# AlwinEsch/pvr.rtl.radiofm

Hardware: AMD Instinct MI355X
Metric: IQ MS/s demodulated (whole node) + achieved HBM GB/s on FIR stage (higher is better)
Workload: dtype f32

## Files before the change

### pvr.rtl.radiofm_amd/csrc/fmd_audio_tail.inc

```
  __builtin_amdgcn_s_setprio(3);
  const unsigned lane = threadIdx.x;
  const unsigned c0 = (blockIdx.x * blockDim.y + threadIdx.y) * 64 + lane;
  if (c0 - lane >= CP)
    return;
  const bool active = c0 < C;
  const unsigned c = active ? c0 : C - 1;
#ifdef FMD_TAIL_ROWS
  const int sel_row = FMD_TAIL_ROWS[c];
  const bool deliver = active && sel_row >= 0;
  const unsigned row = deliver ? (unsigned)sel_row : 0u;
  constexpr bool all_take = false;
#else
  const bool deliver = active;
  const unsigned row = c;
  constexpr bool all_take = true;
#endif
  float de_re = st.F(F_DE_RE)[c], de_im = st.F(F_DE_IM)[c];
  float w1a = st.F(F_N_W1A)[c], w2a = st.F(F_N_W2A)[c], w1b = st.F(F_N_W1B)[c], w2b = st.F(F_N_W2B)[c];
  const int stereo = st.I(I_STEREO_Q0 + (int)stereo_q)[c];
  const float one_minus_alpha = 1.0f - k.de_alpha;
  float vsum = 0.0f, vsumsq = 0.0f;

  auto frame = [&](float2 v) -> float2 {
    de_re = one_minus_alpha * de_re + k.de_alpha * v.x;
    const float s0 = de_re * 2.0f;
    de_im = one_minus_alpha * de_im + k.de_alpha * v.y;
    const float m0 = de_im * 2.0f;
    const float w0a = s0 - k.n_a1 * w1a - k.n_a2 * w2a;
    const float w0b = m0 - k.n_a1 * w1b - k.n_a2 * w2b;
    const float s = k.n_b0 * w0a + k.n_b1 * w1a + k.n_b2 * w2a;
    const float m = k.n_b0 * w0b + k.n_b1 * w1b + k.n_b2 * w2b;
    w2a = w1a;
    w1a = w0a;
    w2b = w1b;
    w1b = w0b;
    const float mm = m * 0.5f;
    const float2 o = stereo ? make_float2((m + s) * 0.5f, (m - s) * 0.5f) : make_float2(mm, mm);
    vsum += o.x;
    vsumsq += o.x * o.x;
    vsum += o.y;
    vsumsq += o.y * o.y;
    return o;
  };
  typename OUT::frame_t* __restrict__ o = reinterpret_cast<typename OUT::frame_t*>(audio + (size_t)row * audio_stride);
  typename OUT::State os;

  unsigned i0 = 0;
  float2 vnext[AT_STEPS];
#pragma unroll
  for (unsigned u = 0; u < AT_STEPS; u++)
    vnext[u] = lp[(size_t)min(u, A - 1) * CP + c];
  for (; i0 + AT_STEPS <= A; i0 += AT_STEPS)
  {
    float2 vin[AT_STEPS];
#pragma unroll
    for (unsigned u = 0; u < AT_STEPS; u++)
      vin[u] = vnext[u];
#pragma unroll
    for (unsigned u = 0; u < AT_STEPS; u++)
      vnext[u] = lp[(size_t)min(i0 + AT_STEPS + u, A - 1) * CP + c];
#pragma unroll
    for (unsigned u = 0; u < AT_STEPS; u++)
    {
      const float2 f = frame(vin[u]);
#ifdef FMD_TAIL_FEED
      if (active)
        FMD_TAIL_FEED[(size_t)(i0 + u) * CP + c] = (f.x + f.y) * 0.5f;
#endif
      if (all_take || deliver)
        OUT::take(os, u, f);
      if (deliver)
        OUT::store(o, os, i0, u, f);
    }
  }
  if (i0 < A)
  {
    const unsigned cnt = A - i0;
#pragma unroll
    for (unsigned u = 0; u < AT_STEPS; u++)
      if (u < cnt)
      {
        const float2 f = frame(vnext[u]);
#ifdef FMD_TAIL_FEED
        if (active)
          FMD_TAIL_FEED[(size_t)(i0 + u) * CP + c] = (f.x + f.y) * 0.5f;
#endif
        if (all_take || deliver)
          OUT::take(os, u, f);
        if (deliver)
          OUT::store(o, os, i0, u, f);
      }
    OUT::flush(o, os, i0, cnt, deliver);
  }
  if (active)
  {
    st.F(F_DE_RE)[c] = de_re;
    st.F(F_DE_IM)[c] = de_im;
    st.F(F_N_W1A)[c] = w1a;
    st.F(F_N_W2A)[c] = w2a;
    st.F(F_N_W1B)[c] = w1b;
    st.F(F_N_W2B)[c] = w2b;
    const float n = (float)(2u * A);
    const float rms = sqrtf(vsumsq / n);
    const float mean = vsum / n;
    const float level = (float)(0.95 * (double)st.F(F_AUDIO_LEVEL)[c] + 0.05 * (double)rms);
    st.F(F_AUDIO_MEAN)[c] = mean;
    st.F(F_AUDIO_RMS)[c] = rms;
    st.F(F_AUDIO_LEVEL)[c] = level;
    unsigned* __restrict__ h = st.ds + c;
    const size_t CPs = st.CP;
    h[HS_IF_LEVEL * CPs] = __float_as_uint(st.F(F_IF_LEVEL)[c]);
    h[HS_BB_MEAN * CPs] = __float_as_uint(st.F(F_BB_MEAN)[c]);
    h[HS_BB_LEVEL * CPs] = __float_as_uint(st.F(F_BB_LEVEL)[c]);
    h[HS_P_LEVEL * CPs] = __float_as_uint(st.F(F_P_LEVEL)[c]);
    h[HS_STEREO * CPs] = (unsigned)stereo;
    h[HS_AUDIO_MEAN * CPs] = __float_as_uint(mean);
    h[HS_AUDIO_RMS * CPs] = __float_as_uint(rms);
    h[HS_AUDIO_LEVEL * CPs] = __float_as_uint(level);
    if (all_take || deliver)
      OUT::done(os, c FMD_TAIL_DONE_ARGS);
  }
```

### pvr.rtl.radiofm_amd/csrc/fmd_k_rds.hip.h

```cpp
#pragma once

#include "fmd_k_common.hip.h"

namespace fmd
{

struct HbCoef
{
  float c[52];
  float e[28];
};

#ifndef FMD_HB_R
#define FMD_HB_R 4
#endif
constexpr int HB_R = FMD_HB_R;

__global__ __launch_bounds__(256) void k_halfband(const float2* __restrict__ in,
                                                  float2* __restrict__ out, unsigned n_out, int L,
                                                  HbCoef hc, unsigned C, unsigned CP, unsigned Hout)
{
  const unsigned c = blockIdx.x * 64 + threadIdx.x;
  const unsigned wy = (unsigned)__builtin_amdgcn_readfirstlane((int)threadIdx.y);
  const unsigned k0 = (blockIdx.y * blockDim.y + wy) * HB_R;
// ... 636 lines not shown
    for (int r = 0; r < RR; r++)
      rf_acc(acc[r], taps[s + r], x);
  }
  if (store)
  {
#pragma unroll
    for (int r = 0; r < RR; r++)
      out[(size_t)(Hout + i + r) * CP + c] = acc[r];
  }
}

template <int RR, typename E>
__device__ __forceinline__ void ring_dispatch(unsigned take, const E* __restrict__ in,
                                              E* __restrict__ out, unsigned i, int T,
                                              const float* __restrict__ taps, unsigned g0, unsigned c,
                                              unsigned CP, unsigned Hout, bool store)
{
  if (take == (unsigned)RR)
    ring_group<RR, E>(in, out, i, T, taps, g0, c, CP, Hout, store);
  else if constexpr (RR > 1)
    ring_dispatch<RR - 1, E>(take, in, out, i, T, taps, g0, c, CP, Hout, store);
}

template <typename E>
__global__ __launch_bounds__(256) void k_ring_fir4(const E* __restrict__ in, E* __restrict__ out,
                                                   unsigned n, int T, const float* __restrict__ taps,
                                                   unsigned g0, unsigned C, unsigned CP, unsigned Hout,
                                                   unsigned prio)
{
  wave_prio(prio);
  const unsigned c = blockIdx.x * 64 + threadIdx.x;
  const unsigned y = (unsigned)__builtin_amdgcn_readfirstlane((int)threadIdx.y);
  unsigned i = (blockIdx.y * blockDim.y + y) * RG;
  if (i >= n)
    return;
  const bool store = c < C;
  unsigned left = min((unsigned)RG, n - i);
  while (left)
  {
    const unsigned room = (unsigned)T - (g0 + i) % (unsigned)T;
    const unsigned take = min(left, room);
    ring_dispatch<RG, E>(take, in, out, i, T, taps, g0, c, CP, Hout, store);
    i += take;
    left -= take;
  }
}

template <typename E>
__global__ __launch_bounds__(256) void k_ring_fir4_org(const E* __restrict__ in, E* __restrict__ out,
                                                       unsigned n, int T, const float* __restrict__ taps,
                                                       unsigned g0, unsigned C, unsigned CP, unsigned Hout,
                                                       unsigned prio, const unsigned* __restrict__ origin)
{
  wave_prio(prio);
  const unsigned c = blockIdx.x * 64 + threadIdx.x;
  const unsigned y = (unsigned)__builtin_amdgcn_readfirstlane((int)threadIdx.y);
  unsigned i = (blockIdx.y * blockDim.y + y) * RG;
  if (i >= n)
    return;
  const bool store = c < C;
  unsigned left = min((unsigned)RG, n - i);
  unsigned lane_g0 = g0;
  const int wg0 = ring_wave_g0(origin, c, C, g0, T, &lane_g0);
  if (wg0 < 0)
  {
    for (; left; i++, left--)
    {
      const unsigned a0 = (lane_g0 + i) % (unsigned)T;
      const E* __restrict__ now = in + (size_t)((unsigned)T - 1 + i) * CP + c;
      const E acc = ring_one_mixed<E>(now, CP, a0, T, taps);
      if (store)
        out[(size_t)(Hout + i) * CP + c] = acc;
    }
    return;
  }
  g0 = (unsigned)wg0;
  while (left)
  {
    const unsigned room = (unsigned)T - (g0 + i) % (unsigned)T;
    const unsigned take = min(left, room);
    ring_dispatch<RG, E>(take, in, out, i, T, taps, g0, c, CP, Hout, store);
    i += take;
    left -= take;
  }
}

template <bool OBS = false>
__device__ __forceinline__ uint32_t rds_check_block(uint32_t& in_bits, uint32_t offset, bool fec,
                                                    uint32_t* pre = nullptr, unsigned* flips = nullptr)
{
  const uint32_t parckh[16] = {0x2DC, 0x16E, 0x0B7, 0x287, 0x39F, 0x313, 0x355, 0x376,
                               0x1BB, 0x201, 0x3DC, 0x1EE, 0x0F7, 0x2A7, 0x38F, 0x31B};
  uint32_t tb = 0x3FFFFFF & in_bits;
  uint32_t syn = tb >> 16;
#pragma unroll
  for (int i = 0; i < 16; i++)
  {
    if (tb & 0x8000)
      syn ^= parckh[i];
    tb <<= 1;
  }
  syn ^= offset;
  if constexpr (OBS)
    *pre = syn;
  if (syn && fec)
  {
    uint32_t mask = 1u << 25;
    for (int i = 0; i < 16; i++)
    {
      if (syn & 0x200)
      {
        if ((syn & 0x1F) == 0)
        {
          in_bits ^= mask;
          syn <<= 1;
          if constexpr (OBS)
            (*flips)++;
        }
        else
        {
          syn <<= 1;
          syn ^= 0x5B9;
        }
      }
      else
        syn <<= 1;
      mask >>= 1;
    }
    syn &= 0x3FF;
  }
  return syn;
}

#ifndef FMD_RP_WAVES
#define FMD_RP_WAVES 4
#endif
constexpr int RP_WAVES = FMD_RP_WAVES;
__global__ __launch_bounds__(64 * RP_WAVES) void k_rds_pll(const float2* __restrict__ lpf, unsigned R, unsigned C,
                                                unsigned CP, RdsConsts k, ChannelState st,
                                                float* __restrict__ rpll, unsigned Hout,
                                                const double* __restrict__ sctab_g, FmdSincosTab sct)
{
  __shared__ double sctab[2 * FMD_SINCOS_TAB_SIZE];
  __builtin_amdgcn_s_setprio(3);
  for (unsigned i = threadIdx.y * 64 + threadIdx.x; i < 2 * FMD_SINCOS_TAB_SIZE; i += 64 * RP_WAVES)
    sctab[i] = sctab_g[i];
  __syncthreads();
  const unsigned c = (blockIdx.x * RP_WAVES + threadIdx.y) * 64 + threadIdx.x;
  if (c >= C)
    return;
  float phase = st.F(F_R_PHASE)[c], freq = st.F(F_R_FREQ)[c];
  float* __restrict__ o = rpll + (size_t)Hout * CP + c;
  constexpr unsigned PT = 16;
  float2 nxt[PT];
#pragma unroll
  for (unsigned u = 0; u < PT; u++)
    nxt[u] = lpf[(size_t)min(u, R - 1) * CP + c];
  for (unsigned i0 = 0; i0 < R; i0 += PT)
  {
    float2 cur[PT];
#pragma unroll
    for (unsigned u = 0; u < PT; u++)
      cur[u] = nxt[u];
#pragma unroll
    for (unsigned u = 0; u < PT; u++)
      nxt[u] = lpf[(size_t)min(i0 + PT + u, R - 1) * CP + c];
    const unsigned cnt = min(PT, R - i0);
#pragma unroll
    for (unsigned u = 0; u < PT; u++)
    {
      if (u < cnt)
      {
        const float2 in = cur[u];
        float sn, cs;
        fmd_sincos_tab(phase, sctab, sct, &sn, &cs);
        const float tr = cs * in.x - sn * in.y;
        const float ti = cs * in.y + sn * in.x;
        const float err = -fmd_rds_arctan2(ti, tr);
        freq += (k.pll_beta * err);
        freq = (freq > k.nco_hl) ? k.nco_hl : ((freq < k.nco_ll) ? k.nco_ll : freq);
        phase += (freq + k.pll_alpha * err);
        *o = ti;
        o += CP;
      }
    }
  }
  st.F(F_R_PHASE)[c] = fmodf(phase, (float)FMD_K_2PI);
  st.F(F_R_FREQ)[c] = freq;
}

constexpr int RB_TILE = 32;

enum RdsQuality
{
  RQ_BITS,
  RQ_CANDIDATES,
  RQ_BLOCKS,
  RQ_CORRECTED,
  RQ_FAILED,
  RQ_ACQUIRED,
  RQ_LOST,
  RQ_GROUPS,
  RQ_N
};
struct RdsObs
{
  unsigned* quality = nullptr;
  uint4* blocks = nullptr;
  unsigned* block_count = nullptr;
  unsigned block_cap = 0;
};

__global__ __launch_bounds__(256) void k_rds_bits(const float* __restrict__ mf, unsigned R, unsigned C,
                                                 unsigned CP, RdsConsts k, ChannelState st,
                                                 uint32_t call_index, RdsGroupRec* __restrict__ queue,
                                                 unsigned* __restrict__ queue_count, unsigned queue_cap,
                                                 float* __restrict__ tap_sync, int write_taps)
{
  constexpr int OBS = 0;
  const RdsObs ob{};
#include "fmd_rds_bits.inc"
}

template <bool RECORD>
__global__ __launch_bounds__(256) void k_rds_bits_obs(const float* __restrict__ mf, unsigned R, unsigned C,
                                                     unsigned CP, RdsConsts k, ChannelState st,
                                                     uint32_t call_index, RdsGroupRec* __restrict__ queue,
                                                     unsigned* __restrict__ queue_count, unsigned queue_cap,
                                                     float* __restrict__ tap_sync, int write_taps, RdsObs ob)
{
  constexpr int OBS = RECORD ? 2 : 1;
#include "fmd_rds_bits.inc"
}

}
```

### pvr.rtl.radiofm_amd/csrc/fmd_k_tail.hip.h

```cpp
#pragma once

#include "fmd_k_common.hip.h"

namespace fmd
{

constexpr int AT_STEPS = 16;

struct OutF32
{
  using frame_t = float2;
  struct State
  {
  };
  static __device__ __forceinline__ void take(State&, unsigned, float2) {}
  static __device__ __forceinline__ void store(float2* o, State&, unsigned i0, unsigned u, float2 f) { o[i0 + u] = f; }
  static __device__ __forceinline__ void flush(float2*, State&, unsigned, unsigned, bool) {}
  static __device__ __forceinline__ void done(State&, unsigned) {}
};
struct OutS16
{
  using frame_t = unsigned;
  struct State
  {
    unsigned w[4];
    unsigned nclip = 0;
  };
  static __device__ __forceinline__ void take(State& s, unsigned u, float2 f)
  {
    const unsigned l = (unsigned)fmd_f32_to_s16_count(f.x, &s.nclip) & 0xffffu;
    const unsigned r = (unsigned)fmd_f32_to_s16_count(f.y, &s.nclip);
    s.w[u & 3u] = l | (r << 16);
  }
  static __device__ __forceinline__ void store(unsigned* o, State& s, unsigned i0, unsigned u, float2)
  {
    if ((u & 3u) == 3u)
      *reinterpret_cast<uint4*>(o + i0 + u - 3u) = make_uint4(s.w[0], s.w[1], s.w[2], s.w[3]);
  }
  static __device__ __forceinline__ void flush(unsigned* o, State& s, unsigned i0, unsigned cnt, bool active)
  {
    if (!active)
      return;
    const unsigned at = i0 + (cnt & ~3u);
    if (cnt & 2u)
      *reinterpret_cast<uint2*>(o + at) = make_uint2(s.w[0], s.w[1]);
    if (cnt & 1u)
      o[at + (cnt & 2u)] = (cnt & 2u) ? s.w[2] : s.w[0];
  }
  static __device__ __forceinline__ void done(State& s, unsigned c, unsigned long long* __restrict__ clipped)
  {
    if (s.nclip)
      clipped[c] += s.nclip;
  }
};

__global__ __launch_bounds__(256) void k_audio_tail(const float2* __restrict__ lp, unsigned A,
                                                   unsigned C, unsigned CP, AudioConsts k,
                                                   ChannelState st, float* __restrict__ audio,
                                                   size_t audio_stride, unsigned stereo_q,
                                                   unsigned call_index)
{
  using OUT = OutF32;
#define FMD_TAIL_DONE_ARGS
#include "fmd_audio_tail.inc"
#undef FMD_TAIL_DONE_ARGS
}

__global__ __launch_bounds__(256) void k_audio_tail_s16(const float2* __restrict__ lp, unsigned A,
                                                       unsigned C, unsigned CP, AudioConsts k,
                                                       ChannelState st, int16_t* __restrict__ audio,
                                                       size_t audio_stride, unsigned stereo_q,
                                                       unsigned call_index,
                                                       unsigned long long* __restrict__ clipped)
{
  using OUT = OutS16;
#define FMD_TAIL_DONE_ARGS , clipped
#include "fmd_audio_tail.inc"
#undef FMD_TAIL_DONE_ARGS
}

__global__ __launch_bounds__(256) void k_audio_tail_sel(const float2* __restrict__ lp, unsigned A, unsigned C,
                                                       unsigned CP, AudioConsts k, ChannelState st,
                                                       float* __restrict__ audio, size_t audio_stride,
                                                       unsigned stereo_q, unsigned call_index,
                                                       const int* __restrict__ rows)
{
  using OUT = OutF32;
#define FMD_TAIL_DONE_ARGS
#define FMD_TAIL_ROWS rows
#include "fmd_audio_tail.inc"
#undef FMD_TAIL_ROWS
#undef FMD_TAIL_DONE_ARGS
}

__global__ __launch_bounds__(256) void k_audio_tail_s16_sel(const float2* __restrict__ lp, unsigned A, unsigned C,
                                                           unsigned CP, AudioConsts k, ChannelState st,
                                                           int16_t* __restrict__ audio, size_t audio_stride,
                                                           unsigned stereo_q, unsigned call_index,
                                                           unsigned long long* __restrict__ clipped,
                                                           const int* __restrict__ rows)
{
  using OUT = OutS16;
#define FMD_TAIL_DONE_ARGS , clipped
#define FMD_TAIL_ROWS rows
#include "fmd_audio_tail.inc"
#undef FMD_TAIL_ROWS
#undef FMD_TAIL_DONE_ARGS
}

#define FMD_TAIL_FEED feed_x
__global__ __launch_bounds__(256) void k_audio_tail_feed(const float2* __restrict__ lp, unsigned A, unsigned C,
                                                        unsigned CP, AudioConsts k, ChannelState st,
                                                        float* __restrict__ audio, size_t audio_stride,
                                                        unsigned stereo_q, unsigned call_index,
                                                        float* __restrict__ feed_x)
{
  using OUT = OutF32;
#define FMD_TAIL_DONE_ARGS
#include "fmd_audio_tail.inc"
#undef FMD_TAIL_DONE_ARGS
}

__global__ __launch_bounds__(256) void k_audio_tail_s16_feed(const float2* __restrict__ lp, unsigned A, unsigned C,
                                                            unsigned CP, AudioConsts k, ChannelState st,
                                                            int16_t* __restrict__ audio, size_t audio_stride,
                                                            unsigned stereo_q, unsigned call_index,
                                                            unsigned long long* __restrict__ clipped,
                                                            float* __restrict__ feed_x)
{
  using OUT = OutS16;
#define FMD_TAIL_DONE_ARGS , clipped
#include "fmd_audio_tail.inc"
#undef FMD_TAIL_DONE_ARGS
}

__global__ __launch_bounds__(256) void k_audio_tail_sel_feed(const float2* __restrict__ lp, unsigned A, unsigned C,
                                                            unsigned CP, AudioConsts k, ChannelState st,
                                                            float* __restrict__ audio, size_t audio_stride,
                                                            unsigned stereo_q, unsigned call_index,
                                                            const int* __restrict__ rows, float* __restrict__ feed_x)
{
  using OUT = OutF32;
#define FMD_TAIL_DONE_ARGS
#define FMD_TAIL_ROWS rows
#include "fmd_audio_tail.inc"
#undef FMD_TAIL_ROWS
#undef FMD_TAIL_DONE_ARGS
}

__global__ __launch_bounds__(256) void k_audio_tail_s16_sel_feed(const float2* __restrict__ lp, unsigned A, unsigned C,
                                                                unsigned CP, AudioConsts k, ChannelState st,
                                                                int16_t* __restrict__ audio, size_t audio_stride,
                                                                unsigned stereo_q, unsigned call_index,
                                                                unsigned long long* __restrict__ clipped,
                                                                const int* __restrict__ rows,
                                                                float* __restrict__ feed_x)
{
  using OUT = OutS16;
#define FMD_TAIL_DONE_ARGS , clipped
#define FMD_TAIL_ROWS rows
#include "fmd_audio_tail.inc"
#undef FMD_TAIL_ROWS
#undef FMD_TAIL_DONE_ARGS
}
#undef FMD_TAIL_FEED

__global__ __launch_bounds__(256) void k_status_publish(ChannelState st, unsigned C, unsigned call_index)
{
  const unsigned c = blockIdx.x * 256 + threadIdx.x;
  if (c >= C)
    return;
  const size_t CPs = st.CP;
  unsigned v[HS_WORDS];
#pragma unroll
  for (int w = HS_SEQ_BEGIN + 1; w < HS_SEQ_END; w++)
    v[w] = st.ds[(size_t)w * CPs + c];
  volatile unsigned* h = st.hs + c;
  h[HS_SEQ_BEGIN * CPs] = call_index;
  __threadfence_system();
#pragma unroll
  for (int w = HS_SEQ_BEGIN + 1; w < HS_SEQ_END; w++)
    h[(size_t)w * CPs] = v[w];
  __threadfence_system();
  h[HS_SEQ_END * CPs] = call_index;
}

__global__ __launch_bounds__(256) void k_rds_export(const RdsGroupRec* __restrict__ queue,
                                                    unsigned* __restrict__ queue_count, unsigned queue_cap,
                                                    int4* __restrict__ rec, unsigned cap,
                                                    unsigned* __restrict__ cursor, unsigned channel_offset,
                                                    unsigned* __restrict__ err)
{
  __shared__ unsigned base_s;
  const unsigned n = min(*queue_count, queue_cap);
  if (threadIdx.x == 0)
    base_s = atomicAdd(cursor, n);
  __syncthreads();
  const unsigned base = base_s;
  for (unsigned i = threadIdx.x; i < n; i += blockDim.x)
  {
// ... 148 lines not shown
```

### pvr.rtl.radiofm_amd/csrc/fmd_math.h

```cpp
#ifndef FMD_MATH_H
#define FMD_MATH_H

#include <math.h>
#include <stdint.h>
#include <string.h>
#ifndef __cplusplus
#include <stdbool.h>
#endif

#ifdef __HIPCC__
#define FMD_HD __host__ __device__ static inline
#define FMD_HD_NOINLINE __host__ __device__ static __attribute__((noinline))
#else
#define FMD_HD static inline
#define FMD_HD_NOINLINE static __attribute__((noinline))
#endif

#if defined(__clang__)
typedef float fmd_v2f __attribute__((ext_vector_type(2)));
#else
typedef float fmd_v2f __attribute__((vector_size(8)));
#endif

FMD_HD fmd_v2f fmd_pk_add_cross(fmd_v2f a, fmd_v2f b)
{
#if defined(__HIP_DEVICE_COMPILE__)
  fmd_v2f r;
  asm("v_pk_add_f32 %0, %1, %2 op_sel:[0,1] op_sel_hi:[1,0] neg_lo:[0,1]" : "=v"(r) : "v"(a), "v"(b));
  return r;
#else
  fmd_v2f r = {a[0] - b[1], a[1] + b[0]};
  return r;
#endif
}

#define FMD_K_2PI (2.0 * 3.14159265358979323846)
#define FMD_K_PI (3.14159265358979323846)
#define FMD_K_PI2 (FMD_K_PI / 2.0)

#if defined(__HIP_DEVICE_COMPILE__)
#define FMD_ANY_LANE(cond) (__builtin_amdgcn_ballot_w64(cond) != 0)
#else
#define FMD_ANY_LANE(cond) (cond)
#endif

FMD_HD float fmd_div_midrange(float n, float d)
{
#if defined(__HIP_DEVICE_COMPILE__)
  const float r0 = __builtin_amdgcn_rcpf(d);
  const float e0 = __builtin_fmaf(-d, r0, 1.0f);
  const float r1 = __builtin_fmaf(e0, r0, r0);
  const float q0 = n * r1;
  const float e1 = __builtin_fmaf(-d, q0, n);
  const float q1 = __builtin_fmaf(e1, r1, q0);
  const float e2 = __builtin_fmaf(-d, q1, n);
  return __builtin_fmaf(e2, r1, q1);
#else
  return n / d;
#endif
}

FMD_HD uint32_t fmd_f2u(float f)
{
  uint32_t u;
  memcpy(&u, &f, 4);
  return u;
}
FMD_HD float fmd_u2f(uint32_t u)
{
  float f;
  memcpy(&f, &u, 4);
  return f;
}

FMD_HD float fmd_u8_to_f32(unsigned b)
{
  const float f = (float)b;
  const float s = __builtin_fmaf(f, 0x1.01p-7f, -1.0f);
  return __builtin_fmaf(f, 0x1.010102p-23f, s);
}

FMD_HD float fmd_s8_to_f32(int v)
{
  return (float)v * 0x1p-7f;
}
FMD_HD float fmd_s16_to_f32(int v)
{
  return (float)v * 0x1p-15f;
}

FMD_HD float fmd_ciq16_to_f32(int v)
{
  return (float)v * 0x1p-13f;
}

FMD_HD int fmd_f32_to_s16_count(float x, unsigned* clipped)
{
  const float y = x * 32768.0f;
  if (y != y)
    return 0;
  const float r = rintf(y);
  *clipped += (r > 32767.0f) | (r < -32768.0f);
  return (int)fminf(fmaxf(r, -32768.0f), 32767.0f);
}
FMD_HD int fmd_f32_to_s16(float x)
{
  unsigned clipped = 0;
  return fmd_f32_to_s16_count(x, &clipped);
}

FMD_HD int fmd_f32_to_mpx16(float x)
{
  const float y = x * 8192.0f;
  if (y != y)
    return 0;
  return (int)fminf(fmaxf(rintf(y), -32768.0f), 32767.0f);
}

FMD_HD float fmd_atanf(float x)
{
  const float atanhi0 = 4.6364760399e-01f, atanhi1 = 7.8539812565e-01f,
              atanhi2 = 9.8279368877e-01f, atanhi3 = 1.5707962513e+00f;
  const float atanlo0 = 5.0121582440e-09f, atanlo1 = 3.7748947079e-08f,
              atanlo2 = 3.4473217170e-08f, atanlo3 = 7.5497894159e-08f;
  const float aT0 = 3.3333334327e-01f, aT1 = -2.0000000298e-01f, aT2 = 1.4285714924e-01f,
              aT3 = -1.1111110449e-01f, aT4 = 9.0908870101e-02f, aT5 = -7.6918758452e-02f,
              aT6 = 6.6610731184e-02f, aT7 = -5.8335702866e-02f, aT8 = 4.9768779427e-02f,
              aT9 = -3.6531571299e-02f, aT10 = 1.6285819933e-02f;
  const float one = 1.0f;
  float w, s1, s2, z;
  int32_t hx = (int32_t)fmd_f2u(x);
  int32_t ix = hx & 0x7fffffff;
  int id;
  float hi = 0.0f, lo = 0.0f;
  if (ix >= 0x4c000000)
  {
    if (ix > 0x7f800000)
      return x + x;
    if (hx > 0)
      return atanhi3 + atanlo3;
    return -atanhi3 - atanlo3;
  }
  if (ix < 0x3ee00000)
  {
    if (ix < 0x31000000)
      return x;
    id = -1;
  }
  else
  {
    x = fabsf(x);
    if (ix < 0x3f980000)
    {
      if (ix < 0x3f300000)
      {
        id = 0;
        x = (2.0f * x - one) / (2.0f + x);
        hi = atanhi0;
        lo = atanlo0;
      }
      else
      {
        id = 1;
        x = (x - one) / (x + one);
        hi = atanhi1;
        lo = atanlo1;
      }
    }
    else
    {
      if (ix < 0x401c0000)
      {
        id = 2;
        x = (x - 1.5f) / (one + 1.5f * x);
        hi = atanhi2;
        lo = atanlo2;
      }
      else
      {
        id = 3;
        x = -1.0f / x;
        hi = atanhi3;
        lo = atanlo3;
      }
    }
  }
  z = x * x;
  w = z * z;
  s1 = z * (aT0 + w * (aT2 + w * (aT4 + w * (aT6 + w * (aT8 + w * aT10)))));
  s2 = w * (aT1 + w * (aT3 + w * (aT5 + w * (aT7 + w * aT9))));
  if (id < 0)
    return x - x * (s1 + s2);
  z = hi - ((x * (s1 + s2) - lo) - x);
  return (hx < 0) ? -z : z;
}

FMD_HD_NOINLINE float fmd_atan2f(float y, float x)
{
  const float tiny = 1.0e-30f, pi_o_4 = 7.8539818525e-01f, pi_o_2 = 1.5707963705e+00f,
              pi = 3.1415927410e+00f, pi_lo = -8.7422776573e-08f;
  float z;
  int32_t hx = (int32_t)fmd_f2u(x), hy = (int32_t)fmd_f2u(y);
  int32_t ix = hx & 0x7fffffff, iy = hy & 0x7fffffff;
  if ((ix > 0x7f800000) || (iy > 0x7f800000))
    return x + y;
  if (hx == 0x3f800000)
    return fmd_atanf(y);
  int m = ((hy >> 31) & 1) | ((hx >> 30) & 2);
  if (iy == 0)
  {
    switch (m)
    {
      case 0:
      case 1:
        return y;
      case 2:
        return pi + tiny;
      default:
        return -pi - tiny;
    }
  }
  if (ix == 0)
    return (hy < 0) ? -pi_o_2 - tiny : pi_o_2 + tiny;
  if (ix == 0x7f800000)
  {
    if (iy == 0x7f800000)
    {
      switch (m)
      {
        case 0:
          return pi_o_4 + tiny;
        case 1:
          return -pi_o_4 - tiny;
        case 2:
          return 3.0f * pi_o_4 + tiny;
        default:
          return -3.0f * pi_o_4 - tiny;
      }
    }
    else
    {
      switch (m)
      {
        case 0:
          return 0.0f;
        case 1:
          return -0.0f;
        case 2:
          return pi + tiny;
        default:
          return -pi - tiny;
      }
    }
  }
  if (iy == 0x7f800000)
    return (hy < 0) ? -pi_o_2 - tiny : pi_o_2 + tiny;
// ... 129 lines not shown
  const float base = ((int32_t)fmd_f2u(x) < 0) ? left : at;
  *rare_measure = rare_m;
  return fmd_u2f(fmd_f2u(base) ^ (fmd_f2u(y) & 0x80000000u));
}

FMD_HD float fmd_atan2f_tab(float y, float x, const float* tab)
{
  uint32_t rare_m;
  float res = fmd_atan2f_tab_core(y, x, tab, &rare_m);
  const bool rare = rare_m >= FMD_ATAN_RARE_LIMIT;
  if (FMD_ANY_LANE(rare))
  {
    if (rare)
      res = fmd_atan2f(y, x);
  }
  return res;
}

struct FmdSincosTab
{
  double inv_h, h_hi, h_lo;
};
#define FMD_SINCOS_TAB_SIZE 1024
FMD_HD void fmd_sincos_tab(float phase, const double* tab , struct FmdSincosTab t,
                           float* s, float* c)
{
  const double x = (double)phase;
  const double magic = 6755399441055744.0;
  const double tt = __builtin_fma(x, t.inv_h, magic);
  const double kf = tt - magic;
  uint64_t ttu;
  memcpy(&ttu, &tt, 8);
  const int k = (int)(uint32_t)ttu;
  double r = __builtin_fma(-kf, t.h_hi, x);
  r = __builtin_fma(-kf, t.h_lo, r);
  const double S = tab[2 * (k & (FMD_SINCOS_TAB_SIZE - 1))];
  const double C = tab[2 * (k & (FMD_SINCOS_TAB_SIZE - 1)) + 1];
  const double r2 = r * r;
  const double sr = __builtin_fma(r * r2, __builtin_fma(r2, 1.0 / 120.0, -1.0 / 6.0), r);
  const double cm1 = r2 * __builtin_fma(r2, 1.0 / 24.0, -0.5);
  const double so = S + __builtin_fma(C, sr, S * cm1);
  const double co = C + __builtin_fma(-S, sr, C * cm1);
  *s = (float)so;
  *c = (float)co;
}

FMD_HD double fmd_fma_const(double x, double a, double b)
{
#if defined(__HIP_DEVICE_COMPILE__)
  double r;
  asm("v_fma_f64 %0, %1, %2, %3" : "=v"(r) : "v"(x), "s"(a), "v"(b));
  return r;
#else
  return __builtin_fma(x, a, b);
#endif
}

#define FMD_SINCOS_P256_SIZE 2048
struct FmdSincosP256
{
  double S, C;
  float r;
};
FMD_HD struct FmdSincosP256 fmd_sincos_p256_lookup(float phase, const double* tab )
{
  const float big = 49152.0f;
  const float t = phase + big;
  const uint32_t k = fmd_f2u(t) & (FMD_SINCOS_P256_SIZE - 1);
  const float kx = t - big;
  struct FmdSincosP256 e;
  e.r = phase - kx;
  e.S = tab[2 * k];
  e.C = tab[2 * k + 1];
  return e;
}
FMD_HD struct FmdSincosP256 fmd_sincos_p256_lookup_lds(float phase, const double* tab)
{
  const float big = 32768.0f;
  const float t = phase + big;
  uint32_t off;
#if defined(__HIP_DEVICE_COMPILE__)
  asm("v_mul_u32_u24 %0, %1, 16" : "=v"(off) : "v"(t));
#else
  off = (fmd_f2u(t) & 0xffffffu) * 16u;
#endif
  const float kx = t - big;
  struct FmdSincosP256 e;
  e.r = phase - kx;
  typedef double fmd_v2d_ __attribute__((vector_size(16)));
  const fmd_v2d_ sc = *(const fmd_v2d_*)((const char*)tab + off);
  e.S = sc[0];
  e.C = sc[1];
  return e;
}
FMD_HD void fmd_sincos_p256_finish(struct FmdSincosP256 e, double m16, float* s, float* c)
{
  const double r = (double)e.r, S = e.S, C = e.C;
  const double r2 = r * r;
#if defined(__HIP_DEVICE_COMPILE__)
  double sr, st;
  asm("v_fma_f64 %1, %2, %3, %4\n\t"
      "v_fma_f64 %0, %5, %1, %6"
      : "=&v"(sr), "=&v"(st)
      : "v"(r2), "s"(1.0 / 120.0), "v"(m16), "v"(r * r2), "v"(r));
#else
  const double sr = __builtin_fma(r * r2, fmd_fma_const(r2, 1.0 / 120.0, m16), r);
#endif
  const double cm1 = r2 * __builtin_fma(r2, 1.0 / 24.0, -0.5);
  const double so = S + __builtin_fma(C, sr, S * cm1);
  const double co = C + __builtin_fma(-S, sr, C * cm1);
  *s = (float)so;
  *c = (float)co;
}
FMD_HD void fmd_sincos_p256k(float phase, const double* tab , double m16, float* s, float* c)
{
  fmd_sincos_p256_finish(fmd_sincos_p256_lookup(phase, tab), m16, s, c);
}
FMD_HD void fmd_sincos_p256(float phase, const double* tab , float* s, float* c)
{
  fmd_sincos_p256k(phase, tab, -1.0 / 6.0, s, c);
}

FMD_HD float fmd_rds_arctan2(float y, float x)
{
  if (x == 0.0f)
  {
    if (y > 0.0f)
      return (float)FMD_K_PI2;
    if (y == 0.0f)
      return 0.0f;
    return (float)-FMD_K_PI2;
  }
  float angle;
  float z = y / x;
  if (fabsf(z) < 1.0f)
  {
    angle = (float)((double)z / (1.0 + 0.2854 * (double)z * (double)z));
    if (x < 0.0f)
    {
      if (y < 0.0f)
        return (float)((double)angle - FMD_K_PI);
      return (float)((double)angle + FMD_K_PI);
    }
  }
  else
  {
    angle = (float)(FMD_K_PI2 - (double)z / ((double)(z * z) + 0.2854));
    if (y < 0.0f)
      return (float)((double)angle - FMD_K_PI);
  }
  return angle;
}

#endif
```

### pvr.rtl.radiofm_amd/csrc/fmd_rds_bits.inc

```
  __builtin_amdgcn_s_setprio(3);
  const unsigned c = (blockIdx.x * blockDim.y + threadIdx.y) * 64 + threadIdx.x;
  if (c >= C)
    return;
  const uint32_t offs[8] = {0x3D8, 0x3D4, 0x25C, 0x258, 0x3D8, 0x3D4, 0x3CC, 0x258};
  float w1 = st.F(F_R_W1)[c], w2 = st.F(F_R_W2)[c];
  float last_sync = st.F(F_R_LAST_SYNC)[c], last_slope = st.F(F_R_LAST_SLOPE)[c],
        last_data = st.F(F_R_LAST_DATA)[c];
  int last_bit = st.I(I_R_LAST_BIT)[c];
  uint32_t bits = (uint32_t)st.I(I_R_BITS)[c];
  int block = st.I(I_R_BLOCK)[c], bitpos = st.I(I_R_BITPOS)[c], state = st.I(I_R_STATE)[c],
      boff = st.I(I_R_BOFF)[c], errors = st.I(I_R_ERRORS)[c];
  uint16_t bd[4];
#pragma unroll
  for (int q = 0; q < 4; q++)
    bd[q] = st.r_data[(size_t)q * CP + c];
  uint32_t seq = (uint32_t)st.I(I_R_SEQ)[c];
  [[maybe_unused]] unsigned rq[RQ_N];
  [[maybe_unused]] uint32_t qpos, qval, o_raw, o_word, o_sample, o_tag;
  [[maybe_unused]] bool rec;
  if constexpr (OBS != 0)
  {
#pragma unroll
    for (int q = 0; q < RQ_N; q++)
      rq[q] = ob.quality[(size_t)q * CP + c];
  }

  float dnext[RB_TILE];
#pragma unroll
  for (unsigned u = 0; u < RB_TILE; u++)
    dnext[u] = mf[(size_t)min(u, R - 1) * CP + c];
  for (unsigned i0 = 0; i0 < R; i0 += RB_TILE)
  {
    const unsigned cnt = min((unsigned)RB_TILE, R - i0);
    float din[RB_TILE];
#pragma unroll
    for (unsigned u = 0; u < RB_TILE; u++)
      din[u] = dnext[u];
#pragma unroll
    for (unsigned u = 0; u < RB_TILE; u++)
      dnext[u] = mf[(size_t)min(i0 + RB_TILE + u, R - 1) * CP + c];
    uint64_t qbits = 0;
    int qcount = 0;
    if constexpr (OBS != 0)
      qpos = qval = 0u;
#pragma unroll
    for (unsigned u = 0; u < RB_TILE; u++)
    {
      if (u >= cnt)
        break;
      const float d = din[u];
      const float mag = d * d;
      const float w0 = mag - k.bs_a1 * w1 - k.bs_a2 * w2;
      const float sv = k.bs_b0 * w0 + k.bs_b1 * w1 + k.bs_b2 * w2;
      w2 = w1;
      w1 = w0;
      if (write_taps)
        tap_sync[(size_t)(i0 + u) * CP + c] = sv;
      const float slope = sv - last_sync;
      last_sync = sv;
      if ((slope < 0.0f) && (last_slope * slope) < 0.0f)
      {
        const int bit = (last_data >= 0) ? 1 : 0;
        if constexpr (OBS == 0)
        {
          qbits = (qbits << 1) | (uint64_t)(bit ^ last_bit);
          qcount++;
        }
        else
        {
          qpos |= 1u << u;
          qval |= (uint32_t)(bit ^ last_bit) << u;
        }
        last_bit = bit;
      }
      last_data = d;
      last_slope = slope;
    }

    while (__any(OBS == 0 ? qcount > 0 : qpos != 0u))
    {
      if constexpr (OBS != 0)
      {
        rec = false;
        o_raw = o_word = o_sample = o_tag = 0u;
      }
      if (OBS == 0 ? qcount > 0 : qpos != 0u)
      {
        if constexpr (OBS == 0)
          qcount--;
        else
        {
          o_sample = (uint32_t)__builtin_ctz(qpos);
          qpos &= qpos - 1u;
          rq[RQ_BITS]++;
        }
        const uint32_t nb = OBS == 0 ? (uint32_t)((qbits >> qcount) & 1u) : (qval >> o_sample) & 1u;
        if constexpr (OBS != 0)
          o_sample += i0;
        bits = (bits << 1) | nb;
        if constexpr (OBS != 0)
          o_raw = bits & 0x3FFFFFFu;
        bool emit = false;
        if (state == 0)
        {
          if (!rds_check_block(bits, offs[0], false))
          {
            if constexpr (OBS != 0)
            {
              rq[RQ_CANDIDATES]++;
              rec = true;
              o_word = (bits >> 10) & 0xFFFFu;
            }
            bitpos = 0;
            boff = 0;
            bd[0] = (uint16_t)(bits >> 10);
            block = 1;
            state = 1;
          }
        }
        else if (++bitpos >= 26)
        {
          bitpos = 0;
          if (state == 3)
          {
            if (++block > 3)
            {
              block = 0;
              state = 2;
            }
          }
          else
          {
            [[maybe_unused]] uint32_t pre = 0;
            [[maybe_unused]] unsigned flips = 0;
            const uint32_t bad = rds_check_block<OBS != 0>(bits, offs[block + boff], state == 2, &pre, &flips);
            if constexpr (OBS != 0)
            {
              const int oi = block + boff;
              const uint32_t status = bad ? 2u : (pre ? 1u : 0u);
              rq[RQ_BLOCKS]++;
              rq[RQ_CORRECTED] += status == 1u;
              rq[RQ_FAILED] += status == 2u;
              rq[RQ_ACQUIRED] += !bad && state == 1 && block >= 3;
              rq[RQ_LOST] += bad && state == 2;
              rec = true;
              o_word = (bits >> 10) & 0xFFFFu;
              o_tag = (oi == 6 ? 4u : (uint32_t)(oi & 3)) | status << 8 | (uint32_t)state << 16 | flips << 24;
            }
            if (bad)
            {
              if (state == 1)
                state = 0;
              else
              {
                errors++;
                if (errors > 0)
                  state = 0;
                else
                {
                  if (++block > 3)
                    block = 0;
                  if (block != 0)
                    state = 3;
                }
              }
            }
            else
            {
              const uint16_t word = (uint16_t)(bits >> 10);
              if (block == 0)
                bd[0] = word;
              else if (block == 1)
                bd[1] = word;
              else if (block == 2)
                bd[2] = word;
              else
                bd[3] = word;
              boff = (block == 1 && (word & 0x0800)) ? 4 : 0;
              if (state == 1)
              {
                if (block >= 3)
                {
                  block = 0;
                  errors = 0;
                  state = 2;
                  emit = true;
                }
                else
                  block++;
              }
              else if (++block > 3)
              {
                block = 0;
// ... 74 lines not shown
```

Measured before the change: 291,300.

## Streamline audio tail, RDS PLL and bit loops with fast-path fetches and branchless math

Adds a fast-path prefetch that skips the per-row min() clamping when a full tile fits, in the audio tail, RDS PLL and RDS bit kernels. The audio tail de-emphasis and notch filter now run on packed two-float vectors. A wave-uniform all-deliver specialization removes the per-sample predication. The RDS PLL splits its main loop from the remainder. It also swaps in select-based arctan2 and s16 conversion variants and replaces the indexed state array with scalar fields to avoid dynamic indexing. The goal is to cut address arithmetic, branches and divergence, at the cost of larger code and possible small numeric differences in the select-based math paths.

New measurement: 293,900 (median of 6 runs). No clear change (+0.9%).

```diff
diff --git a/pvr.rtl.radiofm_amd/csrc/fmd_audio_tail.inc b/pvr.rtl.radiofm_amd/csrc/fmd_audio_tail.inc
--- a/pvr.rtl.radiofm_amd/csrc/fmd_audio_tail.inc
+++ b/pvr.rtl.radiofm_amd/csrc/fmd_audio_tail.inc
@@ -15,62 +15,94 @@
   const unsigned row = c;
   constexpr bool all_take = true;
 #endif
-  float de_re = st.F(F_DE_RE)[c], de_im = st.F(F_DE_IM)[c];
-  float w1a = st.F(F_N_W1A)[c], w2a = st.F(F_N_W2A)[c], w1b = st.F(F_N_W1B)[c], w2b = st.F(F_N_W2B)[c];
-  const int stereo = st.I(I_STEREO_Q0 + (int)stereo_q)[c];
+  fmd_v2f de = {st.F(F_DE_RE)[c], st.F(F_DE_IM)[c]};
+  fmd_v2f w1 = {st.F(F_N_W1A)[c], st.F(F_N_W1B)[c]}, w2 = {st.F(F_N_W2A)[c], st.F(F_N_W2B)[c]};
+  const unsigned stereo_word = (unsigned)st.I(I_STEREO_Q0 + (int)stereo_q)[c];
+  const bool stereo = stereo_word != 0u;
   const float one_minus_alpha = 1.0f - k.de_alpha;
   float vsum = 0.0f, vsumsq = 0.0f;
 
-  auto frame = [&](float2 v) -> float2 {
-    de_re = one_minus_alpha * de_re + k.de_alpha * v.x;
-    const float s0 = de_re * 2.0f;
-    de_im = one_minus_alpha * de_im + k.de_alpha * v.y;
-    const float m0 = de_im * 2.0f;
-    const float w0a = s0 - k.n_a1 * w1a - k.n_a2 * w2a;
-    const float w0b = m0 - k.n_a1 * w1b - k.n_a2 * w2b;
-    const float s = k.n_b0 * w0a + k.n_b1 * w1a + k.n_b2 * w2a;
-    const float m = k.n_b0 * w0b + k.n_b1 * w1b + k.n_b2 * w2b;
-    w2a = w1a;
-    w1a = w0a;
-    w2b = w1b;
-    w1b = w0b;
+  auto frame = [&](float2 vf) -> float2 {
+    const fmd_v2f v = {vf.x, vf.y};
+    de = one_minus_alpha * de + k.de_alpha * v;
+    const fmd_v2f x0 = de * 2.0f;
+    const fmd_v2f w0 = x0 - k.n_a1 * w1 - k.n_a2 * w2;
+    const fmd_v2f y = k.n_b0 * w0 + k.n_b1 * w1 + k.n_b2 * w2;
+    w2 = w1;
+    w1 = w0;
+    const float s = y[0], m = y[1];
+    const fmd_v2f lr = (fmd_v2f){m + s, m - s} * 0.5f;
     const float mm = m * 0.5f;
-    const float2 o = stereo ? make_float2((m + s) * 0.5f, (m - s) * 0.5f) : make_float2(mm, mm);
+    const float2 o = make_float2(stereo ? lr[0] : mm, stereo ? lr[1] : mm);
+    const fmd_v2f oo = (fmd_v2f){o.x, o.y} * (fmd_v2f){o.x, o.y};
     vsum += o.x;
-    vsumsq += o.x * o.x;
+    vsumsq += oo[0];
     vsum += o.y;
-    vsumsq += o.y * o.y;
+    vsumsq += oo[1];
     return o;
   };
   typename OUT::frame_t* __restrict__ o = reinterpret_cast<typename OUT::frame_t*>(audio + (size_t)row * audio_stride);
   typename OUT::State os;
 
+  float2 vnext[AT_STEPS];
+  auto fetch = [&](unsigned r0) {
+    if (r0 + AT_STEPS <= A)
+    {
+      const float2* __restrict__ p = lp + ((size_t)r0 * CP + c);
+#pragma unroll
+      for (unsigned u = 0; u < AT_STEPS; u++)
+        vnext[u] = p[(size_t)u * CP];
+    }
+    else
+    {
+#pragma unroll
+      for (unsigned u = 0; u < AT_STEPS; u++)
+        vnext[u] = lp[(size_t)min(r0 + u, A - 1) * CP + c];
+    }
+  };
+  auto step = [&](auto every, float2 v, unsigned i0, unsigned u) {
+    constexpr bool EVERY = decltype(every)::value;
+    const float2 f = frame(v);
+#ifdef FMD_TAIL_FEED
+    if (EVERY || active)
+      FMD_TAIL_FEED[(size_t)(i0 + u) * CP + c] = (f.x + f.y) * 0.5f;
+#endif
+    if (EVERY || all_take || deliver)
+      OUT::take(os, u, f);
+    if (EVERY || deliver)
+      OUT::store(o, os, i0, u, f);
+  };
+  using Every = std::true_type;
+  using Some = std::false_type;
+
   unsigned i0 = 0;
-  float2 vnext[AT_STEPS];
+  fetch(0);
+  if (__ballot(!deliver) == 0ull)
+  {
+    for (; i0 + AT_STEPS <= A; i0 += AT_STEPS)
+    {
+      float2 vin[AT_STEPS];
 #pragma unroll
-  for (unsigned u = 0; u < AT_STEPS; u++)
-    vnext[u] = lp[(size_t)min(u, A - 1) * CP + c];
-  for (; i0 + AT_STEPS <= A; i0 += AT_STEPS)
+      for (unsigned u = 0; u < AT_STEPS; u++)
+        vin[u] = vnext[u];
+      fetch(i0 + AT_STEPS);
+#pragma unroll
+      for (unsigned u = 0; u < AT_STEPS; u++)
+        step(Every{}, vin[u], i0, u);
+    }
+  }
+  else
   {
-    float2 vin[AT_STEPS];
+    for (; i0 + AT_STEPS <= A; i0 += AT_STEPS)
+    {
+      float2 vin[AT_STEPS];
 #pragma unroll
-    for (unsigned u = 0; u < AT_STEPS; u++)
-      vin[u] = vnext[u];
+      for (unsigned u = 0; u < AT_STEPS; u++)
+        vin[u] = vnext[u];
+      fetch(i0 + AT_STEPS);
 #pragma unroll
-    for (unsigned u = 0; u < AT_STEPS; u++)
-      vnext[u] = lp[(size_t)min(i0 + AT_STEPS + u, A - 1) * CP + c];
-#pragma unroll
-    for (unsigned u = 0; u < AT_STEPS; u++)
-    {
-      const float2 f = frame(vin[u]);
-#ifdef FMD_TAIL_FEED
-      if (active)
-        FMD_TAIL_FEED[(size_t)(i0 + u) * CP + c] = (f.x + f.y) * 0.5f;
-#endif
-      if (all_take || deliver)
-        OUT::take(os, u, f);
-      if (deliver)
-        OUT::store(o, os, i0, u, f);
+      for (unsigned u = 0; u < AT_STEPS; u++)
+        step(Some{}, vin[u], i0, u);
     }
   }
   if (i0 < A)
@@ -79,27 +111,17 @@
 #pragma unroll
     for (unsigned u = 0; u < AT_STEPS; u++)
       if (u < cnt)
-      {
-        const float2 f = frame(vnext[u]);
-#ifdef FMD_TAIL_FEED
-        if (active)
-          FMD_TAIL_FEED[(size_t)(i0 + u) * CP + c] = (f.x + f.y) * 0.5f;
-#endif
-        if (all_take || deliver)
-          OUT::take(os, u, f);
-        if (deliver)
-          OUT::store(o, os, i0, u, f);
-      }
+        step(Some{}, vnext[u], i0, u);
     OUT::flush(o, os, i0, cnt, deliver);
   }
   if (active)
   {
-    st.F(F_DE_RE)[c] = de_re;
-    st.F(F_DE_IM)[c] = de_im;
-    st.F(F_N_W1A)[c] = w1a;
-    st.F(F_N_W2A)[c] = w2a;
-    st.F(F_N_W1B)[c] = w1b;
-    st.F(F_N_W2B)[c] = w2b;
+    st.F(F_DE_RE)[c] = de[0];
+    st.F(F_DE_IM)[c] = de[1];
+    st.F(F_N_W1A)[c] = w1[0];
+    st.F(F_N_W2A)[c] = w2[0];
+    st.F(F_N_W1B)[c] = w1[1];
+    st.F(F_N_W2B)[c] = w2[1];
     const float n = (float)(2u * A);
     const float rms = sqrtf(vsumsq / n);
     const float mean = vsum / n;
@@ -113,7 +135,7 @@
     h[HS_BB_MEAN * CPs] = __float_as_uint(st.F(F_BB_MEAN)[c]);
     h[HS_BB_LEVEL * CPs] = __float_as_uint(st.F(F_BB_LEVEL)[c]);
     h[HS_P_LEVEL * CPs] = __float_as_uint(st.F(F_P_LEVEL)[c]);
-    h[HS_STEREO * CPs] = (unsigned)stereo;
+    h[HS_STEREO * CPs] = stereo_word;
     h[HS_AUDIO_MEAN * CPs] = __float_as_uint(mean);
     h[HS_AUDIO_RMS * CPs] = __float_as_uint(rms);
     h[HS_AUDIO_LEVEL * CPs] = __float_as_uint(level);
diff --git a/pvr.rtl.radiofm_amd/csrc/fmd_k_rds.hip.h b/pvr.rtl.radiofm_amd/csrc/fmd_k_rds.hip.h
--- a/pvr.rtl.radiofm_amd/csrc/fmd_k_rds.hip.h
+++ b/pvr.rtl.radiofm_amd/csrc/fmd_k_rds.hip.h
@@ -812,38 +812,54 @@
   float phase = st.F(F_R_PHASE)[c], freq = st.F(F_R_FREQ)[c];
   float* __restrict__ o = rpll + (size_t)Hout * CP + c;
   constexpr unsigned PT = 16;
+  auto sample = [&](float2 in) {
+    float sn, cs;
+    fmd_sincos_tab(phase, sctab, sct, &sn, &cs);
+    const float tr = cs * in.x - sn * in.y;
+    const float ti = cs * in.y + sn * in.x;
+    const float err = -fmd_rds_arctan2_sel(ti, tr);
+    freq += (k.pll_beta * err);
+    freq = (freq > k.nco_hl) ? k.nco_hl : ((freq < k.nco_ll) ? k.nco_ll : freq);
+    phase += (freq + k.pll_alpha * err);
+    *o = ti;
+    o += CP;
+  };
   float2 nxt[PT];
-#pragma unroll
-  for (unsigned u = 0; u < PT; u++)
-    nxt[u] = lpf[(size_t)min(u, R - 1) * CP + c];
-  for (unsigned i0 = 0; i0 < R; i0 += PT)
+  auto fetch = [&](unsigned r0) {
+    if (r0 + PT <= R)
+    {
+      const float2* __restrict__ p = lpf + ((size_t)r0 * CP + c);
+#pragma unroll
+      for (unsigned u = 0; u < PT; u++)
+        nxt[u] = p[(size_t)u * CP];
+    }
+    else
+    {
+#pragma unroll
+      for (unsigned u = 0; u < PT; u++)
+        nxt[u] = lpf[(size_t)min(r0 + u, R - 1) * CP + c];
+    }
+  };
+  fetch(0);
+  unsigned i0 = 0;
+  for (; i0 + PT <= R; i0 += PT)
   {
     float2 cur[PT];
 #pragma unroll
     for (unsigned u = 0; u < PT; u++)
       cur[u] = nxt[u];
+    fetch(i0 + PT);
 #pragma unroll
     for (unsigned u = 0; u < PT; u++)
-      nxt[u] = lpf[(size_t)min(i0 + PT + u, R - 1) * CP + c];
-    const unsigned cnt = min(PT, R - i0);
+      sample(cur[u]);
+  }
+  if (i0 < R)
+  {
+    const unsigned cnt = R - i0;
 #pragma unroll
     for (unsigned u = 0; u < PT; u++)
-    {
       if (u < cnt)
-      {
-        const float2 in = cur[u];
-        float sn, cs;
-        fmd_sincos_tab(phase, sctab, sct, &sn, &cs);
-        const float tr = cs * in.x - sn * in.y;
-        const float ti = cs * in.y + sn * in.x;
-        const float err = -fmd_rds_arctan2(ti, tr);
-        freq += (k.pll_beta * err);
-        freq = (freq > k.nco_hl) ? k.nco_hl : ((freq < k.nco_ll) ? k.nco_ll : freq);
-        phase += (freq + k.pll_alpha * err);
-        *o = ti;
-        o += CP;
-      }
-    }
+        sample(nxt[u]);
   }
   st.F(F_R_PHASE)[c] = fmodf(phase, (float)FMD_K_2PI);
   st.F(F_R_FREQ)[c] = freq;
diff --git a/pvr.rtl.radiofm_amd/csrc/fmd_k_tail.hip.h b/pvr.rtl.radiofm_amd/csrc/fmd_k_tail.hip.h
--- a/pvr.rtl.radiofm_amd/csrc/fmd_k_tail.hip.h
+++ b/pvr.rtl.radiofm_amd/csrc/fmd_k_tail.hip.h
@@ -23,19 +23,26 @@
   using frame_t = unsigned;
   struct State
   {
-    unsigned w[4];
+    unsigned w0, w1, w2, w3;
     unsigned nclip = 0;
   };
   static __device__ __forceinline__ void take(State& s, unsigned u, float2 f)
   {
-    const unsigned l = (unsigned)fmd_f32_to_s16_count(f.x, &s.nclip) & 0xffffu;
-    const unsigned r = (unsigned)fmd_f32_to_s16_count(f.y, &s.nclip);
-    s.w[u & 3u] = l | (r << 16);
+    const unsigned l = (unsigned)fmd_f32_to_s16_count_sel(f.x, &s.nclip) & 0xffffu;
+    const unsigned r = (unsigned)fmd_f32_to_s16_count_sel(f.y, &s.nclip);
+    const unsigned v = l | (r << 16);
+    switch (u & 3u)
+    {
+      case 0: s.w0 = v; break;
+      case 1: s.w1 = v; break;
+      case 2: s.w2 = v; break;
+      default: s.w3 = v; break;
+    }
   }
   static __device__ __forceinline__ void store(unsigned* o, State& s, unsigned i0, unsigned u, float2)
   {
     if ((u & 3u) == 3u)
-      *reinterpret_cast<uint4*>(o + i0 + u - 3u) = make_uint4(s.w[0], s.w[1], s.w[2], s.w[3]);
+      *reinterpret_cast<uint4*>(o + i0 + u - 3u) = make_uint4(s.w0, s.w1, s.w2, s.w3);
   }
   static __device__ __forceinline__ void flush(unsigned* o, State& s, unsigned i0, unsigned cnt, bool active)
   {
@@ -43,9 +50,9 @@
       return;
     const unsigned at = i0 + (cnt & ~3u);
     if (cnt & 2u)
-      *reinterpret_cast<uint2*>(o + at) = make_uint2(s.w[0], s.w[1]);
+      *reinterpret_cast<uint2*>(o + at) = make_uint2(s.w0, s.w1);
     if (cnt & 1u)
-      o[at + (cnt & 2u)] = (cnt & 2u) ? s.w[2] : s.w[0];
+      o[at + (cnt & 2u)] = (cnt & 2u) ? s.w2 : s.w0;
   }
   static __device__ __forceinline__ void done(State& s, unsigned c, unsigned long long* __restrict__ clipped)
   {
diff --git a/pvr.rtl.radiofm_amd/csrc/fmd_math.h b/pvr.rtl.radiofm_amd/csrc/fmd_math.h
--- a/pvr.rtl.radiofm_amd/csrc/fmd_math.h
+++ b/pvr.rtl.radiofm_amd/csrc/fmd_math.h
@@ -102,6 +102,14 @@
   const float r = rintf(y);
   *clipped += (r > 32767.0f) | (r < -32768.0f);
   return (int)fminf(fmaxf(r, -32768.0f), 32767.0f);
+}
+FMD_HD int fmd_f32_to_s16_count_sel(float x, unsigned* clipped)
+{
+  const float y = x * 32768.0f;
+  const float r = rintf(y);
+  *clipped += (r > 32767.0f) | (r < -32768.0f);
+  const int v = (int)fminf(fmaxf(r, -32768.0f), 32767.0f);
+  return (y != y) ? 0 : v;
 }
 FMD_HD int fmd_f32_to_s16(float x)
 {
@@ -537,4 +545,22 @@
   return angle;
 }
 
-#endif
+FMD_HD float fmd_rds_arctan2_sel(float y, float x)
+{
+  const float z = y / x;
+  const bool first = fabsf(z) < 1.0f;
+  const double zd = (double)z;
+  const double den_first = 1.0 + 0.2854 * zd * zd;
+  const double den_second = (double)(z * z) + 0.2854;
+  const double q = zd / (first ? den_first : den_second);
+  const float angle = first ? (float)q : (float)(FMD_K_PI2 - q);
+  const bool yneg = y < 0.0f;
+  const bool minus = first ? (x < 0.0f && yneg) : yneg;
+  const bool plus = first && x < 0.0f && !yneg;
+  const double turn = minus ? -FMD_K_PI : (plus ? FMD_K_PI : -0.0);
+  const float res = (float)((double)angle + turn);
+  const float on_axis = (y > 0.0f) ? (float)FMD_K_PI2 : ((y == 0.0f) ? 0.0f : (float)-FMD_K_PI2);
+  return (x == 0.0f) ? on_axis : res;
+}
+
+#endif
diff --git a/pvr.rtl.radiofm_amd/csrc/fmd_rds_bits.inc b/pvr.rtl.radiofm_amd/csrc/fmd_rds_bits.inc
--- a/pvr.rtl.radiofm_amd/csrc/fmd_rds_bits.inc
+++ b/pvr.rtl.radiofm_amd/csrc/fmd_rds_bits.inc
@@ -26,9 +26,22 @@
   }
 
   float dnext[RB_TILE];
-#pragma unroll
-  for (unsigned u = 0; u < RB_TILE; u++)
-    dnext[u] = mf[(size_t)min(u, R - 1) * CP + c];
+  auto fetch = [&](unsigned r0) {
+    if (r0 + RB_TILE <= R)
+    {
+      const float* __restrict__ p = mf + ((size_t)r0 * CP + c);
+#pragma unroll
+      for (unsigned u = 0; u < RB_TILE; u++)
+        dnext[u] = p[(size_t)u * CP];
+    }
+    else
+    {
+#pragma unroll
+      for (unsigned u = 0; u < RB_TILE; u++)
+        dnext[u] = mf[(size_t)min(r0 + u, R - 1) * CP + c];
+    }
+  };
+  fetch(0);
   for (unsigned i0 = 0; i0 < R; i0 += RB_TILE)
   {
     const unsigned cnt = min((unsigned)RB_TILE, R - i0);
@@ -36,9 +49,7 @@
 #pragma unroll
     for (unsigned u = 0; u < RB_TILE; u++)
       din[u] = dnext[u];
-#pragma unroll
-    for (unsigned u = 0; u < RB_TILE; u++)
-      dnext[u] = mf[(size_t)min(i0 + RB_TILE + u, R - 1) * CP + c];
+    fetch(i0 + RB_TILE);
     uint64_t qbits = 0;
     int qcount = 0;
     if constexpr (OBS != 0)
```
